# Saguaro-Biosciences/image-processing-suite

Measured on AMD Instinct MI355X. Metric: fields-of-view/sec, 2080x2080x5ch illum+seg+feat pipe, higher is better.
Workload: dtype fp32 planes / fp64 QC+features / fp32 CPnet (split-fp16 MFMA, f16x3); 1 GPU; configs[1]: 384-well plate, 1 FOV/well, 2080x2080x5ch, illum->seg->feat; batch_per_gpu=48, H=2080, W=2080, C=5, cellpose_model=nuclei, cpnet_weights=cpnet_nuclei_synth.pt, tiles_per_fov=9, parallelism=fov-sharded x1, scheduler=static per-rank steps, steps_this_rank=30, batches_in_flight_per_gpu=2

## Files before the change

image-processing-suite_amd/csrc/cpx_internal.h:

```cpp
#pragma once
#include <hip/hip_runtime.h>
#include <stdint.h>
#include <stddef.h>
#include <string>
#include <algorithm>
#include "../../include/cpx.h"

constexpr int kWsSlots = 16;

struct cpx_fov_state;

struct cpx_ctx {
  int device = 0;
  hipStream_t own_stream = nullptr;
  hipStream_t stream = nullptr;
  void* ws[kWsSlots] = {nullptr};
  size_t ws_bytes[kWsSlots] = {0};
  unsigned int ws_gen[kWsSlots] = {0};
  int n_cu = 256;
  int qc_H = 0, qc_W = 0;
  unsigned int qc_gen = 0;
  int seg_key[6] = {0, 0, 0, 0, 0, 0};
  unsigned int seg_gen = 0;
  cpx_fov_state* fov = nullptr;
  int rebin_key[4] = {0, 0, 0, 0};
  unsigned int rebin_gen = 0;
  int embed_key[2] = {0, 0};
  unsigned int embed_gen = 0;
  static constexpr int kGlcmEv = 64;
  int glcm_timing = 0, glcm_nev = 0;
  hipEvent_t glcm_ev[kGlcmEv][2] = {};
  static constexpr int kSegEv = 16;
  int seg_timing = 0, seg_nev = 0;
  hipEvent_t seg_ev[kSegEv][4] = {};
  int* seg_cnt[kSegEv] = {};
  int seg_cnt_cap[kSegEv] = {};
  int seg_B[kSegEv] = {}, seg_rounds[kSegEv] = {};
  int seg_K[kSegEv][64] = {};
  long long fe_count_off = -1;
};

void cpx_fov_free(cpx_ctx* ctx);

enum {
  WS_PARTIALS = 0,
  WS_QC_ROWS = 1,
  WS_QC_RINGS = 2,
  WS_QC_MISC = 3,
  WS_MISC = 4,
  WS_FEAT = 5,
  WS_SEG_PCT = 6,
  WS_SEG_TAB = 7,
  WS_SEG_DYN = 8,
  WS_SEG_OBJ = 9,
  WS_SEG_FILL = 10,
  WS_REBIN = 11,
  WS_REBIN_TMP = 12,
  WS_EMBED = 13,
  WS_WATERSHED = 14,
  WS_MISC2 = 15,
};

void cpx_set_error(const char* fmt, ...);
int cpx_hip_fail(hipError_t e, const char* what);
void* cpx_ws(cpx_ctx* ctx, int slot, size_t bytes);

#define CPX_CHECK_HIP(expr)                                  \
  do {                                                       \
    hipError_t _e = (expr);                                  \
    if (_e != hipSuccess) return cpx_hip_fail(_e, #expr);    \
  } while (0)

#define CPX_CHECK_LAUNCH(what)                                       \
  do {                                                               \
    hipError_t _e = hipGetLastError();                               \
    if (_e != hipSuccess) return cpx_hip_fail(_e, what);             \
  } while (0)

#define CPX_REQUIRE(cond, code, ...)      \
  do {                                    \
    if (!(cond)) {                        \
      cpx_set_error(__VA_ARGS__);         \
      return (code);                      \
    }                                     \
  } while (0)

static inline int cpx_div_up(long long a, long long b) { return (int)((a + b - 1) / b); }

template <typename T>
__device__ __forceinline__ T wave_sum(T v) {
#pragma unroll
  for (int off = 32; off > 0; off >>= 1) v += __shfl_xor(v, off, 64);
  return v;
}
template <typename T>
__device__ __forceinline__ T wave_min(T v) {
#pragma unroll
  for (int off = 32; off > 0; off >>= 1) {
    T o = __shfl_xor(v, off, 64);
    v = o < v ? o : v;
  }
  return v;
}
template <typename T>
__device__ __forceinline__ T wave_max(T v) {
#pragma unroll
  for (int off = 32; off > 0; off >>= 1) {
    T o = __shfl_xor(v, off, 64);
    v = o > v ? o : v;
  }
  return v;
}

constexpr int kClaimBroken = 1 << 30;

constexpr int kFeRegMaxLong = 128, kFeRegMaxShort = 120;
constexpr int kFeRegRows = 40;
constexpr int kFeReg1Rows = 80;
constexpr int kFeKS = 12;
constexpr int kFeU = 1;
constexpr int kFeLargeThreads = 1024, kFeLargeCells = 20224;
__host__ __device__ constexpr int fe_stride(int bw) { return (bw + 3) & ~1; }
__host__ __device__ constexpr bool fe_fits(int bh, int bw, int threads, int units, int cells) {
  const int nsr = (bh + kFeKS - 1) / kFeKS;
  return (long long)(bh + 2) * fe_stride(bw) <= cells &&
         (long long)((bw + 1) / 2) * nsr <= (long long)threads * units;
}
__host__ __device__ constexpr int fe_reg_class(int bh, int bw, bool& tr) {
  const int mn = bh < bw ? bh : bw, mx = bh < bw ? bw : bh;
  if (mn < 1) return 0;
  if (mx <= 64) { tr = bh > bw; return 1; }
  if (mn <= 64 && mx <= kFeReg1Rows) { tr = bw > bh; return 1; }
  if (mx <= 128 && mn <= 2 * kFeRegRows) { tr = bh > bw; return 2; }
  if (mx <= 128 && mn <= 3 * kFeRegRows) { tr = bh > bw; return 3; }
  return 0;
}
enum { kFeListReg1 = 0, kFeListReg2, kFeListReg3, kFeListLds, kFeListOver, kFeListUnd, kFeListFallback, kFeLists };
struct cpx_fe_lists {
  int* count;
  int2* items;
  long long cap;
  __device__ __forceinline__ int n(int l) const { return count[l]; }
  __device__ __forceinline__ int2 at(int l, int i) const { return items[l * cap + i]; }
  __device__ __forceinline__ void push(int l, int fov, int kobj) const {
    items[l * cap + atomicAdd(&count[l], 1)] = make_int2(fov, kobj);
  }
};
__host__ __device__ constexpr int fe_class(int bh, int bw) {
  bool tr = false;
  const int c = fe_reg_class(bh, bw, tr);
  if (c) return kFeListReg1 + c - 1;
  return fe_fits(bh, bw, kFeLargeThreads / 2, 2 * kFeU, kFeLargeCells) ? kFeListLds : kFeListOver;
}
static_assert(fe_class(kFeRegMaxLong, kFeRegMaxShort) == kFeListReg3 &&
                  fe_fits(kFeRegMaxLong, kFeRegMaxShort, kFeLargeThreads / 2, 2 * kFeU, kFeLargeCells) &&
                  fe_fits(kFeRegMaxShort, kFeRegMaxLong, kFeLargeThreads / 2, 2 * kFeU, kFeLargeCells),
              "register-class masks must fit the LDS screening class");

constexpr int kFastShapeWords = 4096;
__host__ __device__ inline bool cpx_shape_fits(int bh, int bw) {
  return (bh + 4) * ((bw + 4 + 31) >> 5) <= kFastShapeWords;
}
struct cpx_fallback_lists {
  int* shape;
  int* tex;
  int* n_shape;
  int* n_tex;
};
typedef int (*cpx_fallback_fn)(cpx_ctx* ctx, hipStream_t stream, const cpx_fallback_lists& fb,
                               void* arg);
int cpx_flow_error_reg_launch(int n_cu, hipStream_t stream, const int* m0, const float2* dpf, int Dy, int Dx,
                              int ML, const cpx_object* obj, cpx_fe_lists lists, int* ctr, double thr,
                              unsigned char* bad);
int cpx_features_fast(cpx_ctx* ctx, const int32_t* labels_dev, const float* corr_dev, int B, int C,
                      int H, int W, int max_label, int F, const cpx_object* objects_dev,
                      const cpx_fov_objects* hdr_dev, double* feats_dev, cpx_fallback_lists* fb,
                      cpx_fallback_fn fallback, void* fallback_arg);
int cpx_features_pair_fast(cpx_ctx* ctx, const int32_t* labels_dev, const int32_t* tlabels_dev,
                           const float* corr_dev, int B, int C, int H, int W, int max_label, int F,
                           const cpx_object* objects_dev, const cpx_fov_objects* hdr_dev, double* feats_dev,
                           const cpx_object* tobjects_dev, const cpx_fov_objects* thdr_dev, double* tfeats_dev,
                           cpx_fallback_lists* fb, cpx_fallback_lists* tfb);
```

image-processing-suite_amd/csrc/k_expand.hip:

```cpp
#include "cpx_internal.h"
#include "ws_levels.h"

namespace {

constexpr int kT = 256;
constexpr signed char kNone = -128;

constexpr int kColTile = 64;

__device__ __forceinline__ int pack_ft(int dr, int lab) { return (lab << 8) | (dr & 0xff); }
__device__ __forceinline__ int ft_dr(int v) { return (int)(signed char)(v & 0xff); }

__global__ __launch_bounds__(kT) void k_edt_cols(const int* __restrict__ labels, int H, int W,
                                                 int D, int* __restrict__ off) {
  const int fov = blockIdx.z;
  const int col = blockIdx.x * kT + threadIdx.x;
  if (col >= W) return;
  const int r0 = blockIdx.y * kColTile, r1 = min(H, r0 + kColTile);
  const long long base = (long long)fov * H * W + col;
  const int* lab = labels + base;
  int* o = off + base;
  int lv[kColTile], cur[kColTile];
#pragma unroll
  for (int u = 0; u < kColTile; ++u) lv[u] = r0 + u < r1 ? lab[(long long)(r0 + u) * W] : 0;
  int last = -0x40000000, last_l = 0;
  for (int rb = max(0, r0 - D); rb < r0; rb += 8) {
    int hv[8];
#pragma unroll
    for (int u = 0; u < 8; ++u) hv[u] = rb + u < r0 ? lab[(long long)(rb + u) * W] : 0;
#pragma unroll
    for (int u = 0; u < 8; ++u)
      if (rb + u < r0 && hv[u] != 0) {
        last = rb + u;
        last_l = hv[u];
      }
  }
#pragma unroll
  for (int u = 0; u < kColTile; ++u) {
    if (lv[u] != 0) {
      last = r0 + u;
      last_l = lv[u];
    }
    const int du = r0 + u - last;
    cur[u] = du <= D ? pack_ft(-du, last_l) : pack_ft(kNone, 0);
  }
  int next = 0x40000000, next_l = 0;
  for (int rb = min(H, r1 + D) - 1; rb >= r1; rb -= 8) {
    int hv[8];
#pragma unroll
    for (int u = 0; u < 8; ++u) hv[u] = rb - u >= r1 ? lab[(long long)(rb - u) * W] : 0;
#pragma unroll
    for (int u = 0; u < 8; ++u)
      if (rb - u >= r1 && hv[u] != 0) {
        next = rb - u;
        next_l = hv[u];
      }
  }
#pragma unroll
  for (int u = kColTile - 1; u >= 0; --u) {
    if (lv[u] != 0) {
      next = r0 + u;
      next_l = lv[u];
    }
    const int dd = next - (r0 + u);
    const int c = ft_dr(cur[u]);
    const int du = c == kNone ? 0x7fffffff : -c;
    if (dd <= D && dd < du) cur[u] = pack_ft(dd, next_l);
  }
#pragma unroll
  for (int u = 0; u < kColTile; ++u)
    if (r0 + u < r1) o[(long long)(r0 + u) * W] = cur[u];
}

constexpr int kRowsPB = 8;
constexpr int kStageMax = (kRowsPB * (kT + 2 * 127) + kT - 1) / kT;

__global__ __launch_bounds__(kT) void k_edt_rows(const int* __restrict__ nuc, int H, int W, int D,
                                                 const int* __restrict__ off,
                                                 int* __restrict__ cells, int* __restrict__ cyto,
                                                 const float* __restrict__ corr, long long cstride,
                                                 unsigned long long* __restrict__ ring, int ntx, int nty) {
  extern __shared__ int seg[];
  const int fov = blockIdx.z, r0 = blockIdx.y * kRowsPB;
  const int nr = min(kRowsPB, H - r0);
  const int c0 = blockIdx.x * kT;
  const int sw = kT + 2 * D;
  const int c = c0 + threadIdx.x;
  int sv[kStageMax], nv_[kRowsPB];
#pragma unroll
  for (int u = 0; u < kStageMax; ++u) {
    const int i = threadIdx.x + u * kT;
    sv[u] = pack_ft(kNone, 0);
    if (i < nr * sw) {
      const int rr = i / sw, k = i - rr * sw;
      const int cc = c0 - D + k;
      if (cc >= 0 && cc < W) sv[u] = off[((long long)fov * H + r0 + rr) * W + cc];
    }
  }
#pragma unroll
  for (int rr = 0; rr < kRowsPB; ++rr)
    nv_[rr] = (rr < nr && c < W) ? nuc[((long long)fov * H + r0 + rr) * W + c] : 0;
#pragma unroll
  for (int u = 0; u < kStageMax; ++u) {
    const int i = threadIdx.x + u * kT;
    if (i < nr * sw) seg[i] = sv[u];
  }
  __syncthreads();
  if (c >= W) return;
#pragma unroll
  for (int rr = 0; rr < kRowsPB; ++rr) {
    if (rr >= nr) break;
    const int* sr = seg + rr * sw + threadIdx.x;
    unsigned best = 0xffffffffu;
    for (int k = 0; k <= 2 * D; ++k) {
      const int dr = ft_dr(sr[k]), dc = k - D;
      best = min(best, ((unsigned)(dr * dr + dc * dc) << 8) | (unsigned)k);
    }
    const int lab = (int)(best >> 8) <= D * D ? sr[best & 0xffu] >> 8 : 0;
    const long long px = ((long long)fov * H + r0 + rr) * W + c;
    const int nv = nv_[rr];
    if (cells) cells[px] = lab;
    if (cyto) cyto[px] = (nv == 0) ? lab : 0;
    if (ring) {
      const int y = r0 + rr, ly = y % wsl::kT, lx = c % wsl::kT;
      if (ly == 0 || ly == wsl::kT - 1 || lx == 0 || lx == wsl::kT - 1) {
        const long long pix = (long long)y * W + c;
        const unsigned long long v =
            wsl::init_level(wsl::info_of(nv, lab, corr[fov * cstride + pix]), pix);
        const long long tile = ((long long)fov * nty + y / wsl::kT) * ntx + c / wsl::kT;
        wsl::ring_store(ring, tile, ly, lx, v);
      }
    }
  }
}

}

int cpx_expand_labels_ring(cpx_ctx* ctx, const int32_t* nuclei_dev, int B, int H, int W, int distance,
                           int32_t* cells_dev, int32_t* cyto_dev, const float* corr_cell,
                           long long corr_stride, unsigned long long* ring) {
  CPX_REQUIRE(ctx && nuclei_dev && (cells_dev || cyto_dev), CPX_ERR_ARG,
              "cpx_expand_labels: null argument");
  CPX_REQUIRE(B > 0 && B <= 65535 && H > 0 && H <= 65535 && W > 0 && distance >= 0 && distance <= 127,
              CPX_ERR_ARG, "cpx_expand_labels: bad sizes (distance must be <= 127)");
  int* off = (int*)cpx_ws(ctx, WS_FEAT, sizeof(int) * (size_t)B * H * W + 256);
  if (!off) return CPX_ERR_OOM;
  hipLaunchKernelGGL(k_edt_cols, dim3(cpx_div_up(W, kT), cpx_div_up(H, kColTile), B), dim3(kT),
                     0, ctx->stream,
                     (const int*)nuclei_dev, H, W, distance, off);
  CPX_CHECK_LAUNCH("k_edt_cols");
  hipLaunchKernelGGL(k_edt_rows, dim3(cpx_div_up(W, kT), cpx_div_up(H, kRowsPB), B), dim3(kT),
                     sizeof(int) * kRowsPB * (kT + 2 * distance), ctx->stream,
                     (const int*)nuclei_dev, H, W, distance, (const int*)off, cells_dev, cyto_dev,
                     corr_cell, corr_stride, ring, cpx_div_up(W, wsl::kT), cpx_div_up(H, wsl::kT));
  CPX_CHECK_LAUNCH("k_edt_rows");
  return CPX_OK;
}

extern "C" int cpx_expand_labels(cpx_ctx* ctx, const int32_t* nuclei_dev, int B, int H, int W,
                                 int distance, int32_t* cells_dev, int32_t* cyto_dev) {
  return cpx_expand_labels_ring(ctx, nuclei_dev, B, H, W, distance, cells_dev, cyto_dev, nullptr, 0, nullptr);
}
```

image-processing-suite_amd/csrc/k_objects.hip:

```cpp
#include "cpx_internal.h"
#include <limits.h>
#include <math.h>

namespace {

constexpr int kThreads = 256;

__global__ void k_stats_init(cpx_label_stats* __restrict__ st, long long n,
                             cpx_fov_objects* __restrict__ hdr, int B) {
  long long i = (long long)blockIdx.x * blockDim.x + threadIdx.x;
  if (i < n) {
    cpx_label_stats s;
    s.area = s.sum_r = s.sum_c = s.sum_rr = s.sum_cc = s.sum_rc = 0;
    s.rmin = INT_MAX;
    s.rmax = -1;
    s.cmin = INT_MAX;
    s.cmax = -1;
    st[i] = s;
  }
  if (i < B) hdr[i] = cpx_fov_objects{0, 0, 0, 0};
}

constexpr int kTileR = 128;
constexpr int kHash = 256;

struct LdsStat {
  int key;
  unsigned int area, sum_r;
  int rmin, rmax, cmin, cmax;
  unsigned int sum_c;
  unsigned long long sum_rr, sum_cc, sum_rc;
};

__device__ __forceinline__ void lds_flush_run(LdsStat* tab, cpx_label_stats* st, int label, int c,
                                              int r0, int r1) {
  const long long cnt = r1 - r0 + 1;
  const long long sr = (long long)(r0 + r1) * cnt / 2;
  const long long srr = ((long long)r1 * (r1 + 1) * (2LL * r1 + 1) -
                         (long long)(r0 - 1) * r0 * (2LL * r0 - 1)) / 6;
  unsigned int h = ((unsigned int)label * 2654435761u) >> 24;
  for (int probe = 0; probe < kHash; ++probe, h = (h + 1) & (kHash - 1)) {
    const int k = atomicCAS(&tab[h].key, 0, label);
    if (k == 0 || k == label) {
      LdsStat* e = tab + h;
      atomicAdd(&e->area, (unsigned int)cnt);
      atomicAdd(&e->sum_r, (unsigned int)sr);
      atomicAdd(&e->sum_c, (unsigned int)(cnt * c));
      atomicAdd(&e->sum_rr, (unsigned long long)srr);
      atomicAdd(&e->sum_cc, (unsigned long long)(cnt * c * c));
      atomicAdd(&e->sum_rc, (unsigned long long)(sr * c));
      atomicMin(&e->rmin, r0);
      atomicMax(&e->rmax, r1);
      atomicMin(&e->cmin, c);
      atomicMax(&e->cmax, c);
      return;
    }
  }
  cpx_label_stats* s = st + label;
  atomicAdd((unsigned long long*)&s->area, (unsigned long long)cnt);
  atomicAdd((unsigned long long*)&s->sum_r, (unsigned long long)sr);
  atomicAdd((unsigned long long*)&s->sum_c, (unsigned long long)(cnt * c));
  atomicAdd((unsigned long long*)&s->sum_rr, (unsigned long long)srr);
  atomicAdd((unsigned long long*)&s->sum_cc, (unsigned long long)(cnt * c * c));
  atomicAdd((unsigned long long*)&s->sum_rc, (unsigned long long)(sr * c));
  atomicMin(&s->rmin, r0);
  atomicMax(&s->rmax, r1);
  atomicMin(&s->cmin, c);
  atomicMax(&s->cmax, c);
}

__global__ __launch_bounds__(kThreads) void k_label_stats(const int* __restrict__ labels, int H,
                                                          int W, int max_label,
                                                          cpx_label_stats* __restrict__ stats,
                                                          cpx_fov_objects* __restrict__ hdr) {
  __shared__ LdsStat tab[kHash];
  const int fov = blockIdx.z;
  {
    LdsStat e;
    e.key = 0;
    e.area = e.sum_r = e.sum_c = 0;
    e.rmin = INT_MAX;
    e.rmax = -1;
    e.cmin = INT_MAX;
    e.cmax = -1;
    e.sum_rr = e.sum_cc = e.sum_rc = 0;
    for (int i = threadIdx.x; i < kHash; i += kThreads) tab[i] = e;
  }
  __syncthreads();
  const int c = blockIdx.x * kThreads + threadIdx.x;
  const int r0 = blockIdx.y * kTileR, r1 = min(H, r0 + kTileR);
  cpx_label_stats* st = stats + (long long)fov * (max_label + 1);
  int seen_max = 0;
  bool overflow = false;
  if (c < W) {
    const int* col = labels + (long long)fov * H * W + c;
    int cur = 0, start = 0;
    for (int rb = r0; rb < r1; rb += 8) {
      int lv[8];
#pragma unroll
      for (int u = 0; u < 8; ++u) lv[u] = rb + u < r1 ? col[(long long)(rb + u) * W] : 0;
#pragma unroll
      for (int u = 0; u < 8; ++u) {
        const int r = rb + u;
        if (r >= r1) break;
        int l = lv[u];
        if (l > 0) {
          seen_max = max(seen_max, l);
          if (l > max_label) {
            overflow = true;
            l = 0;
          }
        }
        if (l != cur) {
          if (cur > 0) lds_flush_run(tab, st, cur, c, start, r - 1);
          cur = l;
          start = r;
        }
      }
    }
    if (cur > 0) lds_flush_run(tab, st, cur, c, start, r1 - 1);
  }
  __syncthreads();
  for (int i = threadIdx.x; i < kHash; i += kThreads) {
    const LdsStat e = tab[i];
    if (e.key == 0) continue;
    cpx_label_stats* s = st + e.key;
    atomicAdd((unsigned long long*)&s->area, (unsigned long long)e.area);
    atomicAdd((unsigned long long*)&s->sum_r, (unsigned long long)e.sum_r);
    atomicAdd((unsigned long long*)&s->sum_c, (unsigned long long)e.sum_c);
    atomicAdd((unsigned long long*)&s->sum_rr, e.sum_rr);
    atomicAdd((unsigned long long*)&s->sum_cc, e.sum_cc);
    atomicAdd((unsigned long long*)&s->sum_rc, e.sum_rc);
    atomicMin(&s->rmin, e.rmin);
    atomicMax(&s->rmax, e.rmax);
    atomicMin(&s->cmin, e.cmin);
    atomicMax(&s->cmax, e.cmax);
  }
  seen_max = wave_max(seen_max);
  int ov = wave_max((int)overflow);
  if ((threadIdx.x & 63) == 0) {
    if (seen_max) atomicMax(&hdr[fov].max_label, seen_max);
    if (ov) atomicMax(&hdr[fov].overflow, 1);
  }
}

__global__ __launch_bounds__(1024) void k_objects_finalize(const cpx_label_stats* __restrict__ stats,
                                                           int H, int W, int max_label, int box,
                                                           cpx_object* __restrict__ objects,
                                                           cpx_fov_objects* __restrict__ hdr) {
  const int fov = blockIdx.x;
  const cpx_label_stats* st = stats + (long long)fov * (max_label + 1);
  cpx_object* out = objects + (long long)fov * max_label;
  __shared__ int wsum_p[16], wsum_k[16];
  __shared__ int base_p, base_k;
  if (threadIdx.x == 0) {
    base_p = 0;
    base_k = 0;
  }
  __syncthreads();
  const int half = box / 2;
  const int lane = threadIdx.x & 63, wid = threadIdx.x >> 6, nw = blockDim.x >> 6;
  for (int l0 = 1; l0 <= max_label; l0 += blockDim.x) {
    const int l = l0 + threadIdx.x;
    int present = 0, kept = 0;
    cpx_label_stats s;
    double cr = 0, cc = 0;
    int yc = 0, xc = 0;
    if (l <= max_label) {
      s = st[l];
      present = s.area > 0;
      if (present) {
        cr = (double)s.sum_r / (double)s.area;
        cc = (double)s.sum_c / (double)s.area;
        yc = (int)cr;
        xc = (int)cc;
        kept = !((yc - half < 0) || (yc + half > H) || (xc - half < 0) || (xc + half > W));
      }
    }
    const unsigned long long bp = __ballot(present), bk = __ballot(kept);
    const unsigned long long lower = (lane == 0) ? 0ull : (~0ull >> (64 - lane));
    const int pre_p = __popcll(bp & lower), pre_k = __popcll(bk & lower);
    if (lane == 0) {
      wsum_p[wid] = __popcll(bp);
      wsum_k[wid] = __popcll(bk);
    }
    __syncthreads();
    int off_p = base_p, off_k = base_k;
    for (int w = 0; w < wid; ++w) {
      off_p += wsum_p[w];
      off_k += wsum_k[w];
    }
    if (present) {
      cpx_object o;
      o.label = l;
      o.area = (int)s.area;
      o.bbox[0] = s.rmin;
      o.bbox[1] = s.cmin;
      o.bbox[2] = s.rmax + 1;
      o.bbox[3] = s.cmax + 1;
      o.centroid_r = cr;
      o.centroid_c = cc;
      o.yc = yc;
      o.xc = xc;
      o.kept = kept;
      o.cell_idx = kept ? off_k + pre_k : -1;
      out[off_p + pre_p] = o;
    }
    __syncthreads();
    if (threadIdx.x == 0) {
      int tp = 0, tk = 0;
      for (int w = 0; w < nw; ++w) {
        tp += wsum_p[w];
        tk += wsum_k[w];
      }
      base_p += tp;
      base_k += tk;
    }
    __syncthreads();
  }
  if (threadIdx.x == 0) {
    hdr[fov].n_objects = base_p;
    hdr[fov].n_kept = base_k;
  }
}

__global__ __launch_bounds__(kThreads) void k_crops(const int* __restrict__ labels,
                                                    const float* __restrict__ corr, int C, int H,
                                                    int W, int max_label,
                                                    const cpx_object* __restrict__ objects,
                                                    const cpx_fov_objects* __restrict__ hdr,
                                                    int box, int max_crops,
                                                    float* __restrict__ crops,
                                                    unsigned char* __restrict__ crops8) {
  const int slot = blockIdx.x, fov = blockIdx.y;
  const cpx_fov_objects h = hdr[fov];
  if (slot >= h.n_kept) return;
  __shared__ int obj_idx;
  if (threadIdx.x == 0) obj_idx = -1;
  __syncthreads();
  const cpx_object* ob = objects + (long long)fov * max_label;
  for (int k = threadIdx.x; k < h.n_objects; k += kThreads)
    if (ob[k].cell_idx == slot) obj_idx = k;
  __syncthreads();
  if (obj_idx < 0) return;
  const cpx_object o = ob[obj_idx];
  const int half = box / 2;
  const int y1 = o.yc - half, x1 = o.xc - half;
  const long long N = (long long)H * W;
  const int* lab = labels + (long long)fov * N;
  const float* img = corr + (long long)fov * C * N;
  const long long npx = (long long)box * box;
  float* dst = crops ? crops + ((long long)fov * max_crops + slot) * npx * C : nullptr;
  __shared__ float smin[8][kThreads / 64], smax[8][kThreads / 64];
  float mn[8], mx[8];
  for (int ch = 0; ch < C && ch < 8; ++ch) {
    mn[ch] = INFINITY;
    mx[ch] = -INFINITY;
  }
  for (long long p = threadIdx.x; p < npx; p += kThreads) {
    const int yy = (int)(p / box), xx = (int)(p % box);
    const long long gi = (long long)(y1 + yy) * W + (x1 + xx);
    const bool in = lab[gi] == o.label;
    for (int ch = 0; ch < C; ++ch) {
      const float v = img[ch * N + gi] * (in ? 1.0f : 0.0f);
      if (dst) dst[p * C + ch] = v;
      if (ch < 8) {
        mn[ch] = fminf(mn[ch], v);
        mx[ch] = fmaxf(mx[ch], v);
      }
    }
  }
  if (!crops8) return;
  const int lane = threadIdx.x & 63, wid = threadIdx.x >> 6;
  for (int ch = 0; ch < C && ch < 8; ++ch) {
    float a = wave_min(mn[ch]), b = wave_max(mx[ch]);
    if (lane == 0) {
      smin[ch][wid] = a;
      smax[ch][wid] = b;
    }
  }
  __syncthreads();
  unsigned char* d8 = crops8 + ((long long)fov * max_crops + slot) * npx * C;
  for (int ch = 0; ch < C && ch < 8; ++ch) {
    float a = smin[ch][0], b = smax[ch][0];
    for (int w = 1; w < kThreads / 64; ++w) {
      a = fminf(a, smin[ch][w]);
      b = fmaxf(b, smax[ch][w]);
    }
    const float rng = b - a;
    for (long long p = threadIdx.x; p < npx; p += kThreads) {
      unsigned char u = 0;
      if (b != a) {
        float v;
        if (dst) {
          v = dst[p * C + ch];
        } else {
          const int yy = (int)(p / box), xx = (int)(p % box);
          const long long gi = (long long)(y1 + yy) * W + (x1 + xx);
          v = img[ch * N + gi] * (lab[gi] == o.label ? 1.0f : 0.0f);
        }
        float t = v - a;
        t = 255.0f * t;
        t = t / rng;
        u = (unsigned char)(int)t;
      }
      d8[(long long)ch * npx + p] = u;
    }
  }
}

}

extern "C" int cpx_objects(cpx_ctx* ctx, const int32_t* labels_dev, int B, int H, int W,
                           int max_label, int box, cpx_label_stats* stats_dev,
                           cpx_object* objects_dev, cpx_fov_objects* hdr_dev) {
  CPX_REQUIRE(ctx && labels_dev && stats_dev && objects_dev && hdr_dev, CPX_ERR_ARG,
              "cpx_objects: null argument");
  CPX_REQUIRE(B > 0 && B <= 65535 && H > 0 && W > 0 && max_label > 0 && box >= 0, CPX_ERR_ARG,
              "cpx_objects: bad sizes");
  const long long nst = (long long)B * (max_label + 1);
  hipLaunchKernelGGL(k_stats_init, dim3(cpx_div_up(std::max<long long>(nst, B), kThreads)),
                     dim3(kThreads), 0, ctx->stream, stats_dev, nst, hdr_dev, B);
  CPX_CHECK_LAUNCH("k_stats_init");
  hipLaunchKernelGGL(k_label_stats, dim3(cpx_div_up(W, kThreads), cpx_div_up(H, kTileR), B),
                     dim3(kThreads), 0, ctx->stream, (const int*)labels_dev, H, W, max_label,
                     stats_dev, hdr_dev);
  CPX_CHECK_LAUNCH("k_label_stats");
  hipLaunchKernelGGL(k_objects_finalize, dim3(B), dim3(1024), 0, ctx->stream,
                     (const cpx_label_stats*)stats_dev, H, W, max_label, box, objects_dev, hdr_dev);
  CPX_CHECK_LAUNCH("k_objects_finalize");
  return CPX_OK;
}

extern "C" int cpx_crops(cpx_ctx* ctx, const int32_t* labels_dev, const float* corr_dev, int B,
                         int C, int H, int W, int max_label, const cpx_object* objects_dev,
                         const cpx_fov_objects* hdr_dev, int box, int max_crops, float* crops_dev,
                         uint8_t* crops8_dev) {
  CPX_REQUIRE(ctx && labels_dev && corr_dev && objects_dev && hdr_dev && (crops_dev || crops8_dev),
              CPX_ERR_ARG, "cpx_crops: null argument");
  CPX_REQUIRE(B > 0 && B <= 65535 && C > 0 && C <= 8 && H > 0 && W > 0 && box > 0 &&
                  max_crops > 0 && max_label > 0,
              CPX_ERR_ARG, "cpx_crops: bad sizes (C must be <= 8)");
  hipLaunchKernelGGL(k_crops, dim3(max_crops, B), dim3(kThreads), 0, ctx->stream,
                     (const int*)labels_dev, corr_dev, C, H, W, max_label, objects_dev, hdr_dev,
                     box, max_crops, crops_dev, (unsigned char*)crops8_dev);
  CPX_CHECK_LAUNCH("k_crops");
  return CPX_OK;
}
```

image-processing-suite_amd/csrc/k_seg.hip:

```cpp
#include "cpx_internal.h"
#include <stdlib.h>
#include <limits.h>
#include <math.h>
#include <stdio.h>
#include <type_traits>
#include <vector>

#pragma clang fp contract(off)

namespace {

constexpr int kT = 256;
constexpr int kRpad = 20;

__device__ __forceinline__ unsigned int f2key(float f) {
  unsigned int u = __float_as_uint(f);
  return (u & 0x80000000u) ? ~u : (u | 0x80000000u);
}
__device__ __forceinline__ float key2f(unsigned int k) {
  unsigned int u = (k & 0x80000000u) ? (k & 0x7fffffffu) : ~k;
  return __uint_as_float(u);
}
__device__ __forceinline__ unsigned short f2bf16(float f) {
  unsigned int u = __float_as_uint(f);
// ... 2251 lines not shown
  return CPX_OK;
}

static int ordered_compact(cpx_ctx* ctx, const unsigned char* flags, long long n, int B, int* tiles,
                           int* totals, int cap, int* out, long long out_stride) {
  const int ntile = cpx_div_up(n, kOcTile);
  hipLaunchKernelGGL(k_oc_count, dim3(ntile, B), dim3(kOcThreads), 0, ctx->stream, flags, n, ntile, tiles);
  hipLaunchKernelGGL(k_oc_scan, dim3(B), dim3(1024), 0, ctx->stream, ntile, tiles, totals);
  hipLaunchKernelGGL(k_oc_emit, dim3(ntile, B), dim3(kOcThreads), 0, ctx->stream, flags, n, ntile,
                     (const int*)tiles, cap, out, out_stride);
  CPX_CHECK_LAUNCH("ordered_compact");
  return CPX_OK;
}

__global__ void k_seed_count(int B, int ms, const int* __restrict__ totals, cpx_seg_stats* __restrict__ st) {
  const int fov = blockIdx.x * blockDim.x + threadIdx.x;
  if (fov >= B) return;
  const int t = totals[fov];
  st[fov].n_seeds = min(t, ms);
  st[fov].n_seeds_found = t;
  if (t > ms) atomicOr(&st[fov].overflow, CPX_SEG_OVF_SEEDS);
}

extern "C" int cpx_seg_masks(cpx_ctx* ctx, const float* yf_dev, int B, const cpx_seg_geom* geom,
                             int H, int W, int niter, double flow_threshold, int min_size,
                             int max_objects, int resample, int32_t* labels_dev,
                             cpx_seg_stats* stats_dev) {
  CPX_REQUIRE(ctx && yf_dev && labels_dev && stats_dev, CPX_ERR_ARG, "cpx_seg_masks: null argument");
  CPX_REQUIRE(geom_ok(geom), CPX_ERR_ARG, "cpx_seg_masks: bad geometry");
  CPX_REQUIRE(B > 0 && B <= 65535 && H > 0 && W > 0 && niter >= 0 && max_objects > 0 &&
                  (long long)(H + 2 * kRpad) * (W + 2 * kRpad) < (1LL << 31) &&
                  (long long)H * W * (long long)sizeof(float2) < (1LL << 32),
              CPX_ERR_ARG, "cpx_seg_masks: bad sizes");
  const int Ly = geom->Ly, Lx = geom->Lx;
  const int Dy = resample ? H : Ly, Dx = resample ? W : Lx;
  const int Dyh = Dy + 2 * kRpad, Dxh = Dx + 2 * kRpad;
  const long long n = (long long)Dy * Dx, nh = (long long)Dyh * Dxh;
  SegTabs tabs;
  int rc = seg_tables(ctx, H, W, Ly, Lx, tabs);
  if (rc) return rc;
  auto al = [](size_t b) { return (b + 255) / 256 * 256; };
  const int ntile = cpx_div_up(std::max(n, nh), kOcTile);
  const size_t sz_f2 = al(sizeof(float2) * B * n);
  const size_t sz_d2 = al(sizeof(float2) * B * n);
  const size_t sz_b = al((size_t)B * n);
  const size_t sz_h = al(sizeof(int) * B * nh), sz_hb = al((size_t)B * nh);
  const size_t sz_m0 = resample ? 0 : al(sizeof(int) * B * n);
  const int ms = max_objects;
  const size_t sz_seeds = al(sizeof(int) * (size_t)B * ms);
  const size_t sz_cnt = al(sizeof(int) * (size_t)B * (ms + 1));
  const size_t sz_act = al(sizeof(int) * B * n);
  const size_t sz_small = al(sizeof(int) * (size_t)B);
  constexpr int k0 = CPX_FOLLOW_K0, sw = 384, k1 = 128;
  const int rounds = cpx_div_up(sw, k0) + cpx_div_up(std::max(0, niter - sw), k1) + 2;
  const size_t sz_fcnt = al(sizeof(int) * (size_t)B * (rounds + 1));
  const size_t sz_items = al((size_t)16 * B * n);
  const size_t sz_tiles = al(sizeof(int) * (size_t)B * ntile);
  const size_t total = sz_d2 + 2 * sz_f2 + 2 * sz_b + 2 * sz_h + sz_hb + sz_m0 + 2 * sz_seeds + 3 * sz_cnt +
                       sz_act + sz_small + sz_tiles + sz_fcnt + 2 * sz_items;
  unsigned char* w = (unsigned char*)cpx_ws(ctx, WS_SEG_DYN, total);
  if (!w) return CPX_ERR_OOM;
  DynBufs d;
  d.dps = (float2*)w; w += sz_d2;
  d.dpf = (float2*)w; w += sz_f2;
  d.p = (float2*)w; w += sz_f2;
  d.mov = w; w += sz_b;
  d.mark = w; w += sz_b;
  d.h = (int*)w; w += sz_h;
  d.M = (unsigned int*)w; w += sz_h;
  d.sflag = w; w += sz_hb;
  d.m0 = resample ? labels_dev : (int*)w; w += sz_m0;
  d.seeds = (int*)w; w += sz_seeds;
  d.marklist = (int*)w; w += sz_seeds;
  d.cnt = (int*)w; w += sz_cnt;
  d.first = (int*)w; w += sz_cnt;
  d.newlab = (int*)w; w += sz_cnt;
  d.act = (int*)w; w += sz_act;
  d.fcnt = (int*)w; w += sz_fcnt;
  d.fitems0 = w; w += sz_items;
  d.fitems1 = w; w += sz_items;
  d.totals = (int*)w; w += sz_small;
  d.tiles = (int*)w; w += sz_tiles;
  d.st = stats_dev;
  d.ms = ms;
  CPX_CHECK_HIP(hipMemsetAsync(stats_dev, 0, sizeof(cpx_seg_stats) * B, ctx->stream));
  CPX_CHECK_HIP(hipMemsetAsync(d.M, 0, sz_h, ctx->stream));
  CPX_CHECK_HIP(hipMemsetAsync(d.mark, 0, sz_b, ctx->stream));
  CPX_CHECK_HIP(hipMemsetAsync(d.cnt, 0, sz_cnt, ctx->stream));
  CPX_CHECK_HIP(hipMemsetAsync(d.first, 0x7f, sz_cnt, ctx->stream));
  CPX_CHECK_HIP(hipMemsetAsync(d.newlab, 0, sz_cnt, ctx->stream));
  CPX_CHECK_HIP(hipMemsetAsync(d.fcnt, 0, sz_fcnt, ctx->stream));
  const dim3 gp(cpx_div_up(n, kT), B), gh(cpx_div_up(nh, kT), B);
  const dim3 gprep(cpx_div_up(n, (long long)kT * kPrepPer), B);
  if (resample)
    hipLaunchKernelGGL(k_dyn_prep<true>, gprep, dim3(kT), 0, ctx->stream, yf_dev, Ly, Lx, Dy, Dx,
                       tabs.uy, tabs.ux, d);
  else
    hipLaunchKernelGGL(k_dyn_prep<false>, gprep, dim3(kT), 0, ctx->stream, yf_dev, Ly, Lx, Dy, Dx,
                       tabs.uy, tabs.ux, d);
  const dim3 gh4(cpx_div_up(nh, (long long)kT * kPx4), B), gp4(cpx_div_up(n, (long long)kT * kPx4), B);
  hipLaunchKernelGGL(k_hist_init, gh4, dim3(kT), 0, ctx->stream, Dy, Dx, d);
  const int sev = ctx->seg_timing && ctx->seg_nev < cpx_ctx::kSegEv ? ctx->seg_nev++ : -1;
  bool fe_timed = false;
  if (sev >= 0) CPX_CHECK_HIP(hipEventRecord(ctx->seg_ev[sev][0], ctx->stream));
  {
    const int fblk = std::max(1, std::min(cpx_div_up(n, kT), (16 * ctx->n_cu + B - 1) / B));
    int step = 0, r = 0;
    do {
      const int K = step < sw ? k0 : k1;
      const FollowItem* in = (const FollowItem*)(r & 1 ? d.fitems1 : d.fitems0);
      FollowItem* out = (FollowItem*)(r & 1 ? d.fitems0 : d.fitems1);
      const bool v4 = Dx >= 2 && 8LL * n < (1LL << 31) && Dy <= (1 << 24) && Dx <= (1 << 24);
      auto kern = v4 ? k_dyn_follow<CPX_FOLLOW_NI, true> : k_dyn_follow<2, false>;
      hipLaunchKernelGGL(kern, dim3(fblk, B), dim3(kT), 0, ctx->stream, Dy, Dx, niter, step, K,
                         r == 0 ? 1 : 0, in, (const int*)(d.fcnt + (size_t)B * r), out,
                         d.fcnt + (size_t)B * (r + 1), d);
      if (sev >= 0 && r < 64) ctx->seg_K[sev][r] = std::min(K, std::max(niter - step, 0));
      step += K;
      ++r;
    } while (step < niter);
    if (sev >= 0) {
      CPX_CHECK_HIP(hipEventRecord(ctx->seg_ev[sev][1], ctx->stream));
      const int rr = std::min(r, 64);
      const int need = B * rr;
      if (ctx->seg_cnt_cap[sev] < need) {
        if (ctx->seg_cnt[sev]) CPX_CHECK_HIP(hipHostFree(ctx->seg_cnt[sev]));
        CPX_CHECK_HIP(hipHostMalloc((void**)&ctx->seg_cnt[sev], sizeof(int) * need));
        ctx->seg_cnt_cap[sev] = need;
      }
      CPX_CHECK_HIP(hipMemcpy2DAsync(ctx->seg_cnt[sev], sizeof(int), stats_dev, sizeof(cpx_seg_stats),
                                     sizeof(int), B, hipMemcpyDeviceToHost, ctx->stream));
      if (rr > 1)
        CPX_CHECK_HIP(hipMemcpyAsync(ctx->seg_cnt[sev] + B, d.fcnt + B, sizeof(int) * B * (rr - 1),
                                     hipMemcpyDeviceToHost, ctx->stream));
      ctx->seg_B[sev] = B;
      ctx->seg_rounds[sev] = rr;
    }
  }
  hipLaunchKernelGGL(k_hist_moving, dim3(1, B), dim3(kT), 0, ctx->stream, Dy, Dx, d);
  hipLaunchKernelGGL(k_seed_flags, gh4, dim3(kT), 0, ctx->stream, Dyh, Dxh, d);
  CPX_CHECK_LAUNCH("cpx_seg_masks follow");
  rc = ordered_compact(ctx, d.sflag, nh, B, d.tiles, d.totals, ms, d.seeds, ms);
  if (rc) return rc;
  hipLaunchKernelGGL(k_seed_count, dim3(cpx_div_up(B, 256)), dim3(256), 0, ctx->stream, B, ms,
                     (const int*)d.totals, stats_dev);
  hipLaunchKernelGGL(k_seed_expand, dim3(std::max(1, (4 * ctx->n_cu + B - 1) / B), B), dim3(kT), 0,
                     ctx->stream, Dyh, Dxh, d);
  hipLaunchKernelGGL(k_assign, dim3(cpx_div_up(n, (long long)kT * kAsg), B), dim3(kT), 0, ctx->stream, Dy, Dx, d);
  hipLaunchKernelGGL(k_relabel_mark, dim3(cpx_div_up(ms, kT), B), dim3(kT), 0, ctx->stream, Dy, Dx, d);
  CPX_CHECK_LAUNCH("cpx_seg_masks seeds");
  rc = ordered_compact(ctx, d.mark, n, B, d.tiles, d.totals, ms, d.marklist, ms);
  if (rc) return rc;
  hipLaunchKernelGGL(k_relabel_apply, dim3(4, B), dim3(kT), 0, ctx->stream, Dy, Dx, d);
  hipLaunchKernelGGL(k_apply_newlab, gp4, dim3(kT), 0, ctx->stream, Dy, Dx, d);
  CPX_CHECK_LAUNCH("cpx_seg_masks relabel");
  const int ML = max_objects;
  const size_t sz_lst = al(sizeof(cpx_label_stats) * (size_t)B * (ML + 1));
  const size_t sz_obj = al(sizeof(cpx_object) * (size_t)B * ML);
  const size_t sz_hdr = al(sizeof(cpx_fov_objects) * (size_t)B);
  const size_t sz_bad = al((size_t)B * (ML + 1));
  const size_t sz_l2i = al(sizeof(int) * (size_t)B * (ML + 1));
  const size_t sz_abs = al(sizeof(int) * (size_t)B * ML);
  const size_t sz_nl = sz_abs;
  constexpr int kFeQueues = 6;
  const size_t sz_fec = al(sizeof(int) * (8 + kFeQueues));
  const size_t sz_fel = al(sizeof(int2) * (size_t)kFeLists * B * ML);
  const size_t gscr_per = (size_t)2 * (Dy + 2) * (Dx + 2);
  const size_t sz_gscr = al(sizeof(double) * B * gscr_per);
  unsigned char* o = (unsigned char*)cpx_ws(ctx, WS_SEG_OBJ,
      sz_lst + sz_obj + sz_hdr + sz_bad + sz_l2i + sz_abs + sz_nl + sz_fec + sz_fel + sz_gscr);
  if (!o) return CPX_ERR_OOM;
  cpx_label_stats* lst = (cpx_label_stats*)o; o += sz_lst;
  cpx_object* obj = (cpx_object*)o; o += sz_obj;
  cpx_fov_objects* hdr = (cpx_fov_objects*)o; o += sz_hdr;
  unsigned char* bad = o; o += sz_bad;
  int* l2i = (int*)o; o += sz_l2i;
  int* absorber = (int*)o; o += sz_abs;
  int* newlab = (int*)o; o += sz_nl;
  int* fec = (int*)o; o += sz_fec;
  int2* fel = (int2*)o; o += sz_fel;
  double* gscr = (double*)o;
  ctx->fe_count_off = -1;
  if (flow_threshold > 0.0) {
    rc = cpx_objects(ctx, d.m0, B, Dy, Dx, ML, 0, lst, obj, hdr);
    if (rc) return rc;
    CPX_CHECK_HIP(hipMemsetAsync(bad, 0, sz_bad, ctx->stream));
    CPX_CHECK_HIP(hipMemsetAsync(fec, 0, sizeof(int) * (8 + kFeQueues), ctx->stream));
    const cpx_fe_lists lists = {fec, fel, (long long)B * ML};
    int* const fq = fec + 8;
    ctx->fe_count_off = (unsigned char*)fec - (unsigned char*)ctx->ws[WS_SEG_OBJ];
    hipLaunchKernelGGL(k_fe_classify, dim3(cpx_div_up(ML, 256), B), dim3(256), 0, ctx->stream, ML,
                       (const cpx_object*)obj, (const cpx_fov_objects*)hdr, lists);
    if (sev >= 0) CPX_CHECK_HIP(hipEventRecord(ctx->seg_ev[sev][2], ctx->stream));
    rc = cpx_flow_error_reg_launch(ctx->n_cu, ctx->stream, d.m0, (const float2*)d.dpf, Dy, Dx, ML, obj, lists,
                                   fq, flow_threshold, bad);
    if (rc) return rc;
    if (sev >= 0) {
      CPX_CHECK_HIP(hipEventRecord(ctx->seg_ev[sev][3], ctx->stream));
      fe_timed = true;
    }
    hipLaunchKernelGGL((k_flow_error_lds<kFeLargeThreads / 2, kFeLargeCells, 2 * kFeU, float, 4>),
                       dim3(2 * ctx->n_cu), dim3(kFeLargeThreads / 2), 0, ctx->stream, (const int*)d.m0,
                       (const float2*)d.dpf, Dy, Dx, ML, (const cpx_object*)obj, lists, fq + 3, flow_threshold,
                       bad);
    hipLaunchKernelGGL(k_flow_error_tail, dim3(ctx->n_cu), dim3(kFeLargeThreads), 0, ctx->stream,
                       (const int*)d.m0, (const float2*)d.dpf, Dy, Dx, ML, (const cpx_object*)obj, lists,
                       fq + 4, flow_threshold, bad);
    {
      const int nbig = std::max(1, std::min(ctx->n_cu, 4 * B));
      const long long slice = (long long)(B * gscr_per / nbig) & ~1LL;
      hipLaunchKernelGGL(k_flow_error_big, dim3(nbig), dim3(kBigThreads), 0, ctx->stream,
                         (const int*)d.m0, (const float2*)d.dpf, Dy, Dx, ML, (const cpx_object*)obj, lists,
                         fq + 5, flow_threshold, gscr, slice, bad);
    }
    hipLaunchKernelGGL(k_flow_error_fov, dim3(B), dim3(kFlowThreads), 0, ctx->stream,
                       (const int*)d.m0, (const float2*)d.dpf, Dy, Dx, ML, (const cpx_object*)obj, lists,
                       flow_threshold, gscr, (long long)gscr_per, bad);
    hipLaunchKernelGGL(k_apply_bad, gp4, dim3(kT), 0, ctx->stream, n, ML,
                       (const unsigned char*)bad, d.m0);
    hipLaunchKernelGGL(k_count_bad, dim3(B), dim3(256), 0, ctx->stream, ML,
                       (const unsigned char*)bad, (const int*)fq, kFeQueues, stats_dev);
    CPX_CHECK_LAUNCH("cpx_seg_masks flow error");
  }
  if (!resample) {
    hipLaunchKernelGGL(k_upsample, dim3(cpx_div_up(W, kT), cpx_div_up(H, kUpRows), B), dim3(kT), 0,
                       ctx->stream, (const int*)d.m0, Ly, Lx, H, W, tabs.ynear, tabs.xnear, labels_dev);
    CPX_CHECK_LAUNCH("k_upsample");
  }
  rc = cpx_objects(ctx, labels_dev, B, H, W, ML, 0, lst, obj, hdr);
  if (rc) return rc;
  const long long N = (long long)H * W;
  const size_t sz_fill = al(sizeof(int) * (size_t)B * N);
  const size_t sz_fscr = al(sizeof(unsigned int) * 2 * (size_t)B * ((W + 31) / 32) * H);
  unsigned char* fw = (unsigned char*)cpx_ws(ctx, WS_SEG_FILL, sz_fill + sz_fscr);
  if (!fw) return CPX_ERR_OOM;
  int* fillidx = (int*)fw;
  unsigned int* fscr = (unsigned int*)(fw + sz_fill);
  CPX_CHECK_HIP(hipMemsetAsync(fillidx, 0, sizeof(int) * (size_t)B * N, ctx->stream));
  CPX_CHECK_HIP(hipMemsetAsync(absorber, 0x7f, sz_abs, ctx->stream));
  CPX_CHECK_HIP(hipMemsetAsync(l2i, 0, sz_l2i, ctx->stream));
  hipLaunchKernelGGL(k_lab2idx, dim3(cpx_div_up(ML, kT), B), dim3(kT), 0, ctx->stream, ML,
                     (const cpx_object*)obj, (const cpx_fov_objects*)hdr, l2i);
  static bool fattr = false;
  const size_t flds = sizeof(unsigned int) * 2 * kFillMaxWords;
  if (!fattr) {
    CPX_CHECK_HIP(hipFuncSetAttribute((const void*)k_fill_holes,
                                      hipFuncAttributeMaxDynamicSharedMemorySize, (int)flds));
    CPX_CHECK_HIP(hipFuncSetAttribute((const void*)k_fill_seq,
                                      hipFuncAttributeMaxDynamicSharedMemorySize, (int)flds));
    fattr = true;
  }
  hipLaunchKernelGGL(k_fill_holes, dim3(std::max(1, std::min(ML, (2 * ctx->n_cu + B - 1) / B)), B),
                     dim3(kFillThreads), flds, ctx->stream,
                     (const int*)labels_dev, H, W, ML, min_size, (const cpx_object*)obj,
                     (const cpx_fov_objects*)hdr, (const int*)l2i, fillidx, absorber);
  hipLaunchKernelGGL(k_fill_holes_big, dim3(B), dim3(1024), 0, ctx->stream,
                     (const int*)labels_dev, H, W, ML, min_size, (const cpx_object*)obj,
                     (const cpx_fov_objects*)hdr, (const int*)l2i, fillidx, absorber, fscr);
  if (sev >= 0 && !fe_timed) {
    CPX_CHECK_HIP(hipEventRecord(ctx->seg_ev[sev][2], ctx->stream));
    CPX_CHECK_HIP(hipEventRecord(ctx->seg_ev[sev][3], ctx->stream));
  }
  hipLaunchKernelGGL(k_fill_final, dim3(B), dim3(1024), 0, ctx->stream, ML, min_size,
                     (const cpx_object*)obj, (const cpx_fov_objects*)hdr, (const int*)absorber,
                     (const int*)labels_dev, (const int*)fillidx, W, N, newlab, stats_dev);
  hipLaunchKernelGGL(k_fill_apply, dim3(std::max(1, std::min(cpx_div_up(N, kT), 8 * ctx->n_cu / B + 1)), B),
                     dim3(kT), 0, ctx->stream, labels_dev, N, ML, (const int*)l2i,
                     (const int*)fillidx, (const int*)newlab, (const int*)absorber,
                     (const cpx_seg_stats*)stats_dev);
  hipLaunchKernelGGL(k_fill_seq, dim3(B), dim3(1024), flds, ctx->stream, labels_dev, H, W, ML, min_size,
                     (const cpx_object*)obj, (const cpx_fov_objects*)hdr, fscr, stats_dev);
  CPX_CHECK_LAUNCH("cpx_seg_masks fill holes");
  return CPX_OK;
}
```

Baseline: 509.4 FOV/s.

## Fuse label remap into object stats and reuse stats after flow-error drop

The separate relabel-apply pass is folded into the label-statistics kernel, which now remaps labels in place while it accumulates stats. When resampling with a flow threshold, the second full-image object scan is replaced by a small kernel that clears the stats of dropped labels and re-finalizes the object table. The EDT expansion kernel also skips the per-pixel nearest-label search for whole waves that have no background pixel or no candidate seed. The aim is to cut full-image passes over label planes, at the cost of more branching and the assumption that stats on the downsampled grid match those the full scan would produce.

Measured after the change: 511.1 FOV/s (median of 6 runs). About the same (+0.3%).

```diff
diff --git a/image-processing-suite_amd/csrc/cpx_internal.h b/image-processing-suite_amd/csrc/cpx_internal.h
--- a/image-processing-suite_amd/csrc/cpx_internal.h
+++ b/image-processing-suite_amd/csrc/cpx_internal.h
@@ -169,6 +169,11 @@
 };
 typedef int (*cpx_fallback_fn)(cpx_ctx* ctx, hipStream_t stream, const cpx_fallback_lists& fb,
                                void* arg);
+int cpx_objects_remap(cpx_ctx* ctx, int32_t* labels_dev, const int* remap_dev, int remap_stride, int B, int H,
+                      int W, int max_label, int box, cpx_label_stats* stats_dev, cpx_object* objects_dev,
+                      cpx_fov_objects* hdr_dev);
+int cpx_objects_refresh(cpx_ctx* ctx, const unsigned char* bad_dev, int B, int H, int W, int max_label, int box,
+                        cpx_label_stats* stats_dev, cpx_object* objects_dev, cpx_fov_objects* hdr_dev);
 int cpx_flow_error_reg_launch(int n_cu, hipStream_t stream, const int* m0, const float2* dpf, int Dy, int Dx,
                               int ML, const cpx_object* obj, cpx_fe_lists lists, int* ctr, double thr,
                               unsigned char* bad);
diff --git a/image-processing-suite_amd/csrc/k_expand.hip b/image-processing-suite_amd/csrc/k_expand.hip
--- a/image-processing-suite_amd/csrc/k_expand.hip
+++ b/image-processing-suite_amd/csrc/k_expand.hip
@@ -106,19 +106,27 @@
     if (i < nr * sw) seg[i] = sv[u];
   }
   __syncthreads();
-  if (c >= W) return;
+  const int lane = threadIdx.x & 63, w0 = threadIdx.x - lane;
+  if (c0 + w0 >= W) return;
+  const bool inb = c < W;
 #pragma unroll
   for (int rr = 0; rr < kRowsPB; ++rr) {
     if (rr >= nr) break;
     const int* sr = seg + rr * sw + threadIdx.x;
-    unsigned best = 0xffffffffu;
-    for (int k = 0; k <= 2 * D; ++k) {
-      const int dr = ft_dr(sr[k]), dc = k - D;
-      best = min(best, ((unsigned)(dr * dr + dc * dc) << 8) | (unsigned)k);
+    const int nv = nv_[rr];
+    bool cand = false;
+    for (int k = lane; k < 64 + 2 * D; k += 64) cand |= ft_dr(seg[rr * sw + w0 + k]) != kNone;
+    int lab = nv;
+    if (__ballot(inb && nv == 0) != 0ull && __ballot(cand) != 0ull) {
+      unsigned best = 0xffffffffu;
+      for (int k = 0; k <= 2 * D; ++k) {
+        const int dr = ft_dr(sr[k]), dc = k - D;
+        best = min(best, ((unsigned)(dr * dr + dc * dc) << 8) | (unsigned)k);
+      }
+      lab = (int)(best >> 8) <= D * D ? sr[best & 0xffu] >> 8 : 0;
     }
-    const int lab = (int)(best >> 8) <= D * D ? sr[best & 0xffu] >> 8 : 0;
+    if (!inb) continue;
     const long long px = ((long long)fov * H + r0 + rr) * W + c;
-    const int nv = nv_[rr];
     if (cells) cells[px] = lab;
     if (cyto) cyto[px] = (nv == 0) ? lab : 0;
     if (ring) {
diff --git a/image-processing-suite_amd/csrc/k_objects.hip b/image-processing-suite_amd/csrc/k_objects.hip
--- a/image-processing-suite_amd/csrc/k_objects.hip
+++ b/image-processing-suite_amd/csrc/k_objects.hip
@@ -1,6 +1,7 @@
 #include "cpx_internal.h"
 #include <limits.h>
 #include <math.h>
+#include <type_traits>
 
 namespace {
 
@@ -69,10 +70,11 @@
   atomicMax(&s->cmax, c);
 }
 
-__global__ __launch_bounds__(kThreads) void k_label_stats(const int* __restrict__ labels, int H,
-                                                          int W, int max_label,
-                                                          cpx_label_stats* __restrict__ stats,
-                                                          cpx_fov_objects* __restrict__ hdr) {
+template <bool REMAP>
+__global__ __launch_bounds__(kThreads) void k_label_stats(
+    typename std::conditional<REMAP, int, const int>::type* __restrict__ labels, int H, int W, int max_label,
+    cpx_label_stats* __restrict__ stats, cpx_fov_objects* __restrict__ hdr, const int* __restrict__ remap,
+    int remap_stride) {
   __shared__ LdsStat tab[kHash];
   const int fov = blockIdx.z;
   {
@@ -93,12 +95,23 @@
   int seen_max = 0;
   bool overflow = false;
   if (c < W) {
-    const int* col = labels + (long long)fov * H * W + c;
+    auto* col = labels + (long long)fov * H * W + c;
     int cur = 0, start = 0;
     for (int rb = r0; rb < r1; rb += 8) {
       int lv[8];
 #pragma unroll
       for (int u = 0; u < 8; ++u) lv[u] = rb + u < r1 ? col[(long long)(rb + u) * W] : 0;
+      if constexpr (REMAP) {
+        const int* rm = remap + (long long)fov * remap_stride;
+        int nv[8];
+#pragma unroll
+        for (int u = 0; u < 8; ++u) nv[u] = lv[u] ? rm[lv[u]] : 0;
+#pragma unroll
+        for (int u = 0; u < 8; ++u) {
+          if (nv[u] != lv[u]) col[(long long)(rb + u) * W] = nv[u];
+          lv[u] = nv[u];
+        }
+      }
 #pragma unroll
       for (int u = 0; u < 8; ++u) {
         const int r = rb + u;
@@ -144,6 +157,39 @@
   }
 }
 
+__global__ __launch_bounds__(kThreads) void k_stats_drop_bad(cpx_label_stats* __restrict__ stats, int max_label,
+                                                             const unsigned char* __restrict__ bad,
+                                                             cpx_fov_objects* __restrict__ hdr) {
+  const int fov = blockIdx.x;
+  cpx_label_stats* st = stats + (long long)fov * (max_label + 1);
+  const unsigned char* bd = bad + (long long)fov * (max_label + 1);
+  __shared__ int smax[kThreads / 64];
+  int mx = 0;
+  for (int l = 1 + threadIdx.x; l <= max_label; l += kThreads) {
+    if (bd[l] == 1) {
+      cpx_label_stats s;
+      s.area = s.sum_r = s.sum_c = s.sum_rr = s.sum_cc = s.sum_rc = 0;
+      s.rmin = INT_MAX;
+      s.rmax = -1;
+      s.cmin = INT_MAX;
+      s.cmax = -1;
+      st[l] = s;
+    } else if (st[l].area > 0) {
+      mx = max(mx, l);
+    }
+  }
+  mx = wave_max(mx);
+  if ((threadIdx.x & 63) == 0) smax[threadIdx.x >> 6] = mx;
+  __syncthreads();
+  if (threadIdx.x == 0) {
+    for (int w = 1; w < kThreads / 64; ++w) mx = max(mx, smax[w]);
+    cpx_fov_objects h = hdr[fov];
+    if (!h.overflow) h.max_label = mx;
+    h.n_objects = h.n_kept = 0;
+    hdr[fov] = h;
+  }
+}
+
 __global__ __launch_bounds__(1024) void k_objects_finalize(const cpx_label_stats* __restrict__ stats,
                                                            int H, int W, int max_label, int box,
                                                            cpx_object* __restrict__ objects,
@@ -311,9 +357,9 @@
 
 }
 
-extern "C" int cpx_objects(cpx_ctx* ctx, const int32_t* labels_dev, int B, int H, int W,
-                           int max_label, int box, cpx_label_stats* stats_dev,
-                           cpx_object* objects_dev, cpx_fov_objects* hdr_dev) {
+static int objects_table(cpx_ctx* ctx, int32_t* labels_dev, const int* remap, int remap_stride, int B, int H,
+                         int W, int max_label, int box, cpx_label_stats* stats_dev, cpx_object* objects_dev,
+                         cpx_fov_objects* hdr_dev) {
   CPX_REQUIRE(ctx && labels_dev && stats_dev && objects_dev && hdr_dev, CPX_ERR_ARG,
               "cpx_objects: null argument");
   CPX_REQUIRE(B > 0 && B <= 65535 && H > 0 && W > 0 && max_label > 0 && box >= 0, CPX_ERR_ARG,
@@ -322,10 +368,44 @@
   hipLaunchKernelGGL(k_stats_init, dim3(cpx_div_up(std::max<long long>(nst, B), kThreads)),
                      dim3(kThreads), 0, ctx->stream, stats_dev, nst, hdr_dev, B);
   CPX_CHECK_LAUNCH("k_stats_init");
-  hipLaunchKernelGGL(k_label_stats, dim3(cpx_div_up(W, kThreads), cpx_div_up(H, kTileR), B),
-                     dim3(kThreads), 0, ctx->stream, (const int*)labels_dev, H, W, max_label,
-                     stats_dev, hdr_dev);
+  const dim3 grid(cpx_div_up(W, kThreads), cpx_div_up(H, kTileR), B);
+  if (remap)
+    hipLaunchKernelGGL(k_label_stats<true>, grid, dim3(kThreads), 0, ctx->stream, (int*)labels_dev, H, W,
+                       max_label, stats_dev, hdr_dev, remap, remap_stride);
+  else
+    hipLaunchKernelGGL(k_label_stats<false>, grid, dim3(kThreads), 0, ctx->stream, (const int*)labels_dev, H, W,
+                       max_label, stats_dev, hdr_dev, (const int*)nullptr, 0);
   CPX_CHECK_LAUNCH("k_label_stats");
+  hipLaunchKernelGGL(k_objects_finalize, dim3(B), dim3(1024), 0, ctx->stream,
+                     (const cpx_label_stats*)stats_dev, H, W, max_label, box, objects_dev, hdr_dev);
+  CPX_CHECK_LAUNCH("k_objects_finalize");
+  return CPX_OK;
+}
+
+extern "C" int cpx_objects(cpx_ctx* ctx, const int32_t* labels_dev, int B, int H, int W,
+                           int max_label, int box, cpx_label_stats* stats_dev,
+                           cpx_object* objects_dev, cpx_fov_objects* hdr_dev) {
+  return objects_table(ctx, const_cast<int32_t*>(labels_dev), nullptr, 0, B, H, W, max_label, box, stats_dev,
+                       objects_dev, hdr_dev);
+}
+
+int cpx_objects_remap(cpx_ctx* ctx, int32_t* labels_dev, const int* remap_dev, int remap_stride, int B, int H,
+                      int W, int max_label, int box, cpx_label_stats* stats_dev, cpx_object* objects_dev,
+                      cpx_fov_objects* hdr_dev) {
+  CPX_REQUIRE(remap_dev && remap_stride > 0, CPX_ERR_ARG, "cpx_objects_remap: null argument");
+  return objects_table(ctx, labels_dev, remap_dev, remap_stride, B, H, W, max_label, box, stats_dev,
+                       objects_dev, hdr_dev);
+}
+
+int cpx_objects_refresh(cpx_ctx* ctx, const unsigned char* bad_dev, int B, int H, int W, int max_label, int box,
+                        cpx_label_stats* stats_dev, cpx_object* objects_dev, cpx_fov_objects* hdr_dev) {
+  CPX_REQUIRE(ctx && bad_dev && stats_dev && objects_dev && hdr_dev, CPX_ERR_ARG,
+              "cpx_objects_refresh: null argument");
+  CPX_REQUIRE(B > 0 && B <= 65535 && H > 0 && W > 0 && max_label > 0 && box >= 0, CPX_ERR_ARG,
+              "cpx_objects_refresh: bad sizes");
+  hipLaunchKernelGGL(k_stats_drop_bad, dim3(B), dim3(kThreads), 0, ctx->stream, stats_dev, max_label, bad_dev,
+                     hdr_dev);
+  CPX_CHECK_LAUNCH("k_stats_drop_bad");
   hipLaunchKernelGGL(k_objects_finalize, dim3(B), dim3(1024), 0, ctx->stream,
                      (const cpx_label_stats*)stats_dev, H, W, max_label, box, objects_dev, hdr_dev);
   CPX_CHECK_LAUNCH("k_objects_finalize");
diff --git a/image-processing-suite_amd/csrc/k_seg.hip b/image-processing-suite_amd/csrc/k_seg.hip
--- a/image-processing-suite_amd/csrc/k_seg.hip
+++ b/image-processing-suite_amd/csrc/k_seg.hip
@@ -2427,7 +2427,7 @@
   rc = ordered_compact(ctx, d.mark, n, B, d.tiles, d.totals, ms, d.marklist, ms);
   if (rc) return rc;
   hipLaunchKernelGGL(k_relabel_apply, dim3(4, B), dim3(kT), 0, ctx->stream, Dy, Dx, d);
-  hipLaunchKernelGGL(k_apply_newlab, gp4, dim3(kT), 0, ctx->stream, Dy, Dx, d);
+  if (!(flow_threshold > 0.0)) hipLaunchKernelGGL(k_apply_newlab, gp4, dim3(kT), 0, ctx->stream, Dy, Dx, d);
   CPX_CHECK_LAUNCH("cpx_seg_masks relabel");
   const int ML = max_objects;
   const size_t sz_lst = al(sizeof(cpx_label_stats) * (size_t)B * (ML + 1));
@@ -2457,7 +2457,7 @@
   double* gscr = (double*)o;
   ctx->fe_count_off = -1;
   if (flow_threshold > 0.0) {
-    rc = cpx_objects(ctx, d.m0, B, Dy, Dx, ML, 0, lst, obj, hdr);
+    rc = cpx_objects_remap(ctx, d.m0, d.newlab, ms + 1, B, Dy, Dx, ML, 0, lst, obj, hdr);
     if (rc) return rc;
     CPX_CHECK_HIP(hipMemsetAsync(bad, 0, sz_bad, ctx->stream));
     CPX_CHECK_HIP(hipMemsetAsync(fec, 0, sizeof(int) * (8 + kFeQueues), ctx->stream));
@@ -2502,7 +2502,10 @@
                        ctx->stream, (const int*)d.m0, Ly, Lx, H, W, tabs.ynear, tabs.xnear, labels_dev);
     CPX_CHECK_LAUNCH("k_upsample");
   }
-  rc = cpx_objects(ctx, labels_dev, B, H, W, ML, 0, lst, obj, hdr);
+  if (resample && flow_threshold > 0.0)
+    rc = cpx_objects_refresh(ctx, bad, B, H, W, ML, 0, lst, obj, hdr);
+  else
+    rc = cpx_objects(ctx, labels_dev, B, H, W, ML, 0, lst, obj, hdr);
   if (rc) return rc;
   const long long N = (long long)H * W;
   const size_t sz_fill = al(sizeof(int) * (size_t)B * N);
```
